# chungimungi/GMLM

Measured on AMD Instinct MI355X. Metric: nodes/sec fwd+bwd (full-batch GraphTextLM step), higher is better.
Workload: dtype bf16; 1 GPU; squirrel-size synthetic graph x1 (N=5201, E=217073, F_in=2089), hidden_channels=768, BERT geometry 768x12, 1257 active text nodes, 16..128 tokens, plm_batch_size=4096; global_nodes=5201, parallelism=single GPU, activation_checkpointing=False, plm_gradient_checkpointing=False, world=1, hip_graph=False, gemm_algorithms=library picks from gmlm_amd/tunable/gfx950.csv (TunableOp lookup)

## Files before the change

gmlm_amd/_lib.py:

```python
from __future__ import annotations

import ctypes as C
import os

_HERE = os.path.dirname(os.path.abspath(__file__))
LIB_PATH = os.path.join(_HERE, "libgmlm_hip.so")

F32, BF16 = 0, 1
_p, _i64, _i32, _f32, _u64, _sz = C.c_void_p, C.c_int64, C.c_int, C.c_float, C.c_uint64, C.c_size_t

SIGNATURES = {
    "gmlm_version": (C.c_int, []),
    "gmlm_last_error": (C.c_char_p, []),
    "gmlm_device_check": (C.c_int, [_p, _p, C.c_char_p, _i32]),
    "gmlm_degree_i32": (C.c_int, [_p, _i64, _i64, _p, _p]),
    "gmlm_degree_f32": (C.c_int, [_p, _i64, _i64, _p, _p]),
    "gmlm_edge_bucket": (C.c_int, [_p, _p, _i64, _i64, _p, _p]),
    "gmlm_relation_histogram": (C.c_int, [_p, _i64, _i32, _p, _p]),
    "gmlm_segment_sort_workspace_bytes": (_sz, [_i64]),
    "gmlm_segment_sort": (C.c_int, [_p, _p, _p, _i32, _i64, _i64, _p, _p, _p, _p, _p, _sz, _p]),
    "gmlm_gather_i64_to_i32": (C.c_int, [_p, _p, _i64, _p, _p]),
    "gmlm_gather_i32": (C.c_int, [_p, _p, _i64, _p, _p]),
    "gmlm_segment_inv_count": (C.c_int, [_p, _i64, _p, _p]),
    "gmlm_split_plan_capacity": (C.c_int, [_i64, _i64, C.POINTER(C.c_int64), C.POINTER(C.c_int64)]),
    "gmlm_split_plan_build": (C.c_int, [_p, _i64, _i64, _i64, _p, _p, _p, _p]),
    "gmlm_rgcn_mean_spmm": (C.c_int, [_p, _i64, _i64, _p, _p, _p, _i32, _i64, _i64, _p, _i64, _i32, _i64, _p, _p, _p, _i64, _i64,
                                      _p, _p]),
    "gmlm_basis_compose_fwd": (C.c_int, [_p, _p, _i32, _i32, _i64, _p, _p]),
    "gmlm_basis_compose_bwd_workspace_bytes": (_sz, [_i32, _i32, _i64]),
    "gmlm_basis_compose_bwd": (C.c_int, [_p, _p, _p, _i32, _i32, _i64, _p, _p, _p, _sz, _p]),
    "gmlm_colstats_workspace_bytes": (_sz, [_i64, _i64]),
    "gmlm_colstats": (C.c_int, [_p, _i32, _p, _i64, _i64, _p, _p, _p, _sz, _p]),
    "gmlm_graphnorm_finalize": (C.c_int, [_p, _p, _p, _p, _i64, _i64, _f32, _p, _p, _p]),
    "gmlm_graphnorm_apply": (C.c_int, [_p, _p, _p, _p, _p, _p, _i64, _i64, _i32, _f32, _u64, _p, _p, _i32, _p]),
    "gmlm_graphnorm_bwd_stats": (C.c_int, [_p, _i32, _p, _p, _p, _p, _p, _p, _i64, _i64, _i32, _f32, _u64, _p, _p, _p, _sz, _p]),
    "gmlm_graphnorm_bwd_apply": (C.c_int, [_p, _i32, _p, _p, _p, _p, _p, _p, _p, _i64, _i64, _i64, _i32, _f32, _u64, _p,
                                           _p, _p, _p, _p, _p]),
    "gmlm_bias_res_layernorm_fwd": (C.c_int, [_p, _p, _p, _p, _p, _i64, _i64, _f32, _i32, _f32, _u64, _p, _p, _p, _p, _i32, _p]),
    "gmlm_layernorm_bwd_workspace_bytes": (_sz, [_i64, _i64]),
    "gmlm_bias_res_layernorm_bwd": (C.c_int, [_p, _p, _p, _p, _p, _p, _p, _p, _i64, _i64, _i32, _f32, _u64, _p, _p, _p, _p, _p,
                                              _p, _i32, _p, _sz, _p]),
    "gmlm_attention_fwd": (C.c_int, [_p, _p, _p, _p, _i64, _i64, _i64, _i64, _i64, _i64, _i64, _i64, _f32, _f32, _u64, _p,
                                     _p, _p, _p, _i32, _p, _i64, _p, _i64, _p]),
    "gmlm_attention_bwd_workspace_bytes": (_sz, [_i64, _i64, _i64, _i64, _i64]),
    "gmlm_attention_bwd": (C.c_int, [_p, _p, _p, _p, _p, _p, _p, _i64, _i64, _i64, _i64, _i64, _i64, _i64, _i64, _f32,
                                     _f32, _u64, _p, _p, _p, _p, _i64, _i64, _i64, _i32, _p, _i64, _p, _sz, _p, _p, _p, _p, _i64, _p]),
    "gmlm_embed_sum_fwd": (C.c_int, [_p, _p, _p, _p, _p, _i64, _i64, _i64, _i64, _p, _i32, _p, _p]),
    "gmlm_meanpool_scatter_fwd": (C.c_int, [_p, _p, _p, _i64, _i64, _i64, _p, _i32, _p, _p]),
    "gmlm_meanpool_scatter_bwd": (C.c_int, [_p, _p, _p, _i64, _i64, _i64, _p, _i32, _p, _p]),
    "gmlm_softmask_blend_fwd": (C.c_int, [_p, _p, _p, _f32, _i64, _i64, _p, _i64, _i32, _p]),
    "gmlm_softmask_blend_bwd": (C.c_int, [_p, _i64, _p, _f32, _i64, _i64, _p, _p, _sz, _p]),
    "gmlm_bias_gelu_fwd": (C.c_int, [_p, _p, _i64, _i64, _f32, _u64, _p, _p, _i32, _p]),
    "gmlm_bias_gelu_bwd_workspace_bytes": (_sz, [_i64, _i64, _i32]),
    "gmlm_bias_gelu_bwd": (C.c_int, [_p, _p, _p, _i64, _i64, _f32, _u64, _p, _p, _p, _i32, _p, _sz, _p]),
}


class GmlmHipError(RuntimeError):
    pass


_lib = None


def lib() -> C.CDLL:
    global _lib
    if _lib is not None:
        return _lib
    if not os.path.exists(LIB_PATH):
        raise GmlmHipError(
            f"{LIB_PATH} not found: the HIP extension is not built. Run `make -C gmlm_amd/csrc` "
            "(or __graft_entry__.build()). gmlm_amd has no CPU / eager fallback.")
    handle = C.CDLL(LIB_PATH)
    for name, (res, args) in SIGNATURES.items():
        fn = getattr(handle, name)
        fn.restype, fn.argtypes = res, args
    if handle.gmlm_version() != 1:
        raise GmlmHipError(f"ABI version mismatch: library {handle.gmlm_version()} != binding 1")
    _lib = handle
    return handle


def check(rc: int, what: str = "") -> None:
    if rc != 0:
        msg = lib().gmlm_last_error().decode(errors="replace")
        raise GmlmHipError(f"{what or 'gmlm call'} failed (code {rc}): {msg}")


_device_ok = {}


def require_gfx950(device_index: int) -> None:
    if _device_ok.get(device_index):
        return
    import torch
    with torch.cuda.device(device_index):
        arch = C.create_string_buffer(64)
        cu, wave = C.c_int(0), C.c_int(0)
        check(lib().gmlm_device_check(C.byref(cu), C.byref(wave), arch, 64), "gmlm_device_check")
    _device_ok[device_index] = (cu.value, wave.value, arch.value.decode())


def device_info(device_index: int = 0):
    require_gfx950(device_index)
    return _device_ok[device_index]
```

gmlm_amd/nn.py:

```python
from __future__ import annotations

import math
from typing import Optional

import torch
import torch.nn as nn
import torch.nn.functional as F

from . import ops
from .graph import GraphCache, RelCSR

_GRAPHS = GraphCache(capacity=8)


def compute_dtype(module_dtype: Optional[torch.dtype] = None) -> torch.dtype:
    if module_dtype is not None:
        return module_dtype
    if torch.is_autocast_enabled("cuda"):
        if torch.get_autocast_dtype("cuda") == torch.float16:
            _warn_fp16_once()
        return torch.bfloat16
    return torch.float32


_FP16_WARNED = False


def _warn_fp16_once() -> None:
    global _FP16_WARNED
    if not _FP16_WARNED:
        _FP16_WARNED = True
        import warnings
        warnings.warn("gmlm_amd: fp16 autocast is executed with bf16 operands (the HIP kernels' reduced precision); "
                      "use torch.amp.autocast('cuda', dtype=torch.bfloat16) to make that explicit", stacklevel=3)


def _glorot(t: torch.Tensor) -> None:
    a = math.sqrt(6.0 / (t.size(-2) + t.size(-1)))
    with torch.no_grad():
        t.uniform_(-a, a)


def _linear(x, weight, bias=None):
    sh = _SHADOW
    if sh is not None and x.dtype == sh.dtype:
        wc = sh.get(id(weight))
        bc = sh.get(id(bias)) if bias is not None else None
        if wc is not None and (bias is None or bc is not None):
            return _mm(x, wc, bc, (weight,) + ((bias,) if bias is not None else ()))
    with torch.autocast("cuda", enabled=False):
        w = weight.to(x.dtype)
        b = None if bias is None else bias.to(x.dtype)
        return F.linear(x, w, b)


_F32_OUT = [True]
_F32_MM = [True]


_SLICES_MEASURED = {(2304, 768): 14, (3072, 768): 14, (768, 3072): 14}
SPLITK_ROW_QUANTUM = 112


def _splitk_wgrad(dy2: torch.Tensor, x2: torch.Tensor, keep_fp32: bool = False) -> torch.Tensor:
    t, n = dy2.shape
    k = x2.shape[1]
    tiles = ((n + 255) // 256) * ((k + 255) // 256)
    s = 1
    if tiles < 128 and t >= 16384:
        import math
        s = _SLICES_MEASURED.get((n, k), 16) if t >= 65536 else min(16, max(1, 2 ** round(math.log2(200.0 / tiles))))
    if s == 1:
        if keep_fp32 and dy2.dtype != torch.float32 and _F32_MM[0]:
            try:
                return torch.mm(dy2.t(), x2, out_dtype=torch.float32)
            except (RuntimeError, TypeError):
                _F32_MM[0] = False
        dw = dy2.t() @ x2
        return dw.float() if keep_fp32 else dw
    q = t // s
    a = dy2[:s * q].view(s, q, n).transpose(1, 2)
    b = x2[:s * q].view(s, q, k)
    if _F32_OUT[0] and dy2.dtype != torch.float32:
        try:
            dw = torch.bmm(a, b, out_dtype=torch.float32).sum(0)
        except (RuntimeError, TypeError):
            _F32_OUT[0] = False
            dw = torch.bmm(a, b).float().sum(0)
    else:
        dw = torch.bmm(a, b).float().sum(0)
    if s * q < t:
        dw += dy2[s * q:].t() @ x2[s * q:]
    return dw if keep_fp32 else dw.to(dy2.dtype)


class _Linear(torch.autograd.Function):

    @staticmethod
    def forward(ctx, x, wc, bc, residual, bias_grad, *masters):
        ctx.save_for_backward(x, wc)
        ctx.masters = masters
        ctx.has_bias = bc is not None and bias_grad
        ctx.n_w = len(masters) // 2 if ctx.has_bias else len(masters)
        y = torch.nn.functional.linear(x, wc, bc)
        return (y, x.view_as(x)) if residual else y

    @staticmethod
    def backward(ctx, dy, dxres=None):
        x, wc = ctx.saved_tensors
        masters, n_w = ctx.masters, ctx.n_w
        dy2 = dy.reshape(-1, dy.shape[-1])
        x2 = x.reshape(-1, x.shape[-1])
        dx = None
        if ctx.needs_input_grad[0]:
            if dxres is None:
                dx = (dy2 @ wc).view(x.shape)
            else:
                dres2 = dxres.reshape(-1, x.shape[-1])
                dx = (dres2.addmm_(dy2, wc) if dres2.is_contiguous() else torch.addmm(dres2, dy2, wc)).view(x.shape)
        grads = [None] * len(masters)
        need = ctx.needs_input_grad[5:]
        if any(need[:n_w]):
            dw = _splitk_wgrad(dy2, x2, keep_fp32=True)
            for i, (m, g) in enumerate(zip(masters[:n_w], dw.split([m.shape[0] for m in masters[:n_w]], 0))):
                if need[i]:
                    grads[i] = g if g.dtype == m.dtype else g.to(m.dtype)
        if ctx.has_bias and any(need[n_w:]):
            db = ops.column_sum(dy2) if dy2.is_cuda and dy2.dtype in (torch.float32, torch.bfloat16) else dy2.sum(0, dtype=torch.float32)
            for i, (m, g) in enumerate(zip(masters[n_w:], db.split([m.shape[0] for m in masters[n_w:]], 0))):
                if need[n_w + i]:
                    grads[n_w + i] = g if g.dtype == m.dtype else g.to(m.dtype)
        return (dx, None, None, None, None, *grads)


def _mm(x, wc, bc, masters, residual=False, bias_grad=True):
    with torch.autocast("cuda", enabled=False):
        return _Linear.apply(x, wc, bc, residual, bias_grad, *masters)


class ParamShadow:

    def __init__(self, specs, dtype, device):
        total, plan = 0, []
        for key, masters, pad in specs:
            rows = sum(m.shape[0] for m in masters) + pad
            tail = tuple(masters[0].shape[1:])
            numel = rows
            for d in tail:
                numel *= d
            plan.append((key, masters, (rows,) + tail, total, numel))
            total += (numel + 127) // 128 * 128
        self.dtype = dtype
        with torch.no_grad():
            flat = torch.zeros(total, dtype=dtype, device=device)
            self.flat = flat
            self.views, dsts, srcs = {}, [], []
            for key, masters, shape, off, numel in plan:
                v = flat[off:off + numel].view(shape)
                self.views[key] = v
                r0 = 0
                for m in masters:
                    dsts.append(v[r0:r0 + m.shape[0]])
                    srcs.append(m.detach())
                    r0 += m.shape[0]
            if dsts:
                torch._foreach_copy_(dsts, srcs)

    def get(self, key):
        return self.views.get(key)

    def record_stream(self, stream) -> None:
        if self.flat.is_cuda:
            self.flat.record_stream(stream)


_SHADOW: Optional[ParamShadow] = None


class shadow_params:

    def __init__(self, specs, dtype, device):
        self.args = (specs, dtype, device)
        self.prev = None

    def __enter__(self):
        global _SHADOW
        self.prev = _SHADOW
        specs, dtype, device = self.args
        _SHADOW = ParamShadow(specs, dtype, device) if (dtype != torch.float32 and device.type == "cuda") else None
        return _SHADOW

    def __exit__(self, *exc):
        global _SHADOW
        _SHADOW = self.prev
        return False


class use_shadow:

    def __init__(self, sh):
        self.sh, self.prev = sh, None

    def __enter__(self):
        global _SHADOW
        self.prev = _SHADOW
        if _SHADOW is None:
            _SHADOW = self.sh
        return _SHADOW

    def __exit__(self, *exc):
        global _SHADOW
        _SHADOW = self.prev
        return False


def linear_specs(*mods):
    out = []
    for m in mods:
        out.append((id(m.weight), [m.weight], 0))
        if m.bias is not None:
            out.append((id(m.bias), [m.bias], 0))
    return out


class _RootAddmm(torch.autograd.Function):

    @staticmethod
    def forward(ctx, x, rootc, bc, root, bias):
        ctx.save_for_backward(x, rootc)
        ctx.rows = root.shape[0]
        return torch.addmm(bc, x, rootc)

    @staticmethod
    def backward(ctx, dy):
        x, rootc = ctx.saved_tensors
        dx = dy @ rootc.t() if ctx.needs_input_grad[0] else None
        droot = _splitk_wgrad(x, dy, keep_fp32=True)[:ctx.rows] if ctx.needs_input_grad[3] else None
        db = ops.column_sum(dy) if ctx.needs_input_grad[4] else None
        return dx, None, None, droot, db


class _SelectRows(torch.autograd.Function):

    @staticmethod
    def forward(ctx, x, idx):
        ctx.save_for_backward(idx)
        ctx.rows = x.shape[0]
        return x.index_select(0, idx)

    @staticmethod
    def backward(ctx, g):
        (idx,) = ctx.saved_tensors
        out = g.new_zeros((ctx.rows,) + tuple(g.shape[1:]))
        out.index_copy_(0, idx, g)
        return out, None


class _BasisCompose(torch.autograd.Function):

    @staticmethod
    def forward(ctx, comp_a, weight2d, reducer):
        comp_a, weight2d = comp_a.detach().float().contiguous(), weight2d.detach().float().contiguous()
        ra, nb = comp_a.shape
        cols = weight2d.shape[1]
        ctx.save_for_backward(comp_a, weight2d)
        ctx.reducer = reducer
        if not weight2d.is_cuda or nb > 32 or ra > 5 or cols % 4:
            if not weight2d.is_cuda:
                raise ops._lib.GmlmHipError("gmlm_amd ops run on the GPU only; there is no CPU path")
            ctx.hip = False
            return comp_a @ weight2d
        ctx.hip = True
        w = torch.empty(ra, cols, dtype=torch.float32, device=weight2d.device)
        ops.check(ops.lib().gmlm_basis_compose_fwd(ops._ptr(comp_a), ops._ptr(weight2d), ra, nb, cols, ops._ptr(w),
                                                   ops._stream()), "gmlm_basis_compose_fwd")
        return w

    @staticmethod
    def backward(ctx, dw):
        comp_a, weight2d = ctx.saved_tensors
        dw = dw.float().contiguous()
        if ctx.reducer is not None:
            ctx.reducer(dw)
        if not ctx.hip:
            return dw @ weight2d.t(), comp_a.t() @ dw, None
        ra, nb = comp_a.shape
        cols = weight2d.shape[1]
        dweight = torch.empty_like(weight2d)
        dcomp = torch.empty_like(comp_a)
        ws = ops._ws(ops.lib().gmlm_basis_compose_bwd_workspace_bytes(ra, nb, cols), dw.device)
        ops.check(ops.lib().gmlm_basis_compose_bwd(ops._ptr(comp_a), ops._ptr(weight2d), ops._ptr(dw), ra, nb, cols,
                                                   ops._ptr(dweight), ops._ptr(dcomp), ops._ptr(ws), ws.numel(), ops._stream()),
                  "gmlm_basis_compose_bwd")
        return dcomp, dweight, None


class RGCNConv(nn.Module):

    def __init__(self, in_channels: int, out_channels: int, num_relations: int, num_bases: Optional[int] = None, **kw):
        super().__init__()
        if kw:
            raise TypeError(f"unsupported RGCNConv options: {sorted(kw)}")
        if num_bases is None:
            raise NotImplementedError("only the basis-decomposed form used by the reference (num_bases=30) is implemented")
        self.in_channels, self.out_channels = in_channels, out_channels
        self.num_relations, self.num_bases = num_relations, num_bases
        self.weight = nn.Parameter(torch.empty(num_bases, in_channels, out_channels))
        self.comp = nn.Parameter(torch.empty(num_relations, num_bases))
        self.root = nn.Parameter(torch.empty(in_channels, out_channels))
        self.bias = nn.Parameter(torch.zeros(out_channels))
        self.reset_parameters()

    def reset_parameters(self):
        _glorot(self.weight), _glorot(self.comp), _glorot(self.root)
        nn.init.zeros_(self.bias)

    def relation_weights(self, csr: RelCSR, dtype, in_pad: int = 0, reducer=None) -> torch.Tensor:
        comp = _SelectRows.apply(self.comp, csr.active_index)
        w = _BasisCompose.apply(comp, self.weight.view(self.num_bases, -1), reducer)
        self.weight._gmlm_grad_reduced = self.comp._gmlm_grad_reduced = reducer is not None
        w = w.view(len(csr.active_relations), self.in_channels, self.out_channels)
        if in_pad:
            w = F.pad(w, (0, 0, 0, in_pad))
        return w.reshape(-1, self.out_channels).to(dtype)

    def forward_csr(self, x: torch.Tensor, csr: RelCSR, reducer=None, halo_wait=None) -> torch.Tensor:
        in_pad = x.shape[1] - self.in_channels
        n = csr.num_nodes
        sh = _SHADOW
        rootc = sh.get(id(self.root)) if (sh is not None and x.dtype == sh.dtype) else None
        bc = sh.get(id(self.bias)) if rootc is not None else None
        with torch.autocast("cuda", enabled=False):
            w = self.relation_weights(csr, x.dtype, in_pad, reducer)
            if bc is not None and rootc.shape[0] == x.shape[1]:
                out = _RootAddmm.apply(x if x.shape[0] == n else x[:n], rootc, bc, self.root, self.bias)
            else:
                root = self.root if not in_pad else F.pad(self.root, (0, 0, 0, in_pad))
                out = torch.addmm(self.bias.to(x.dtype), x[:n], root.to(x.dtype))
        if halo_wait is not None:
            x = halo_wait(x)
        h = ops.RGCNAggregate.apply(x, csr)
        with torch.autocast("cuda", enabled=False):
            return out.addmm_(h, w)

    def forward(self, x, edge_index, edge_type):
        csr = _GRAPHS.get(edge_index, x.size(0), self.num_relations, edge_type)
        cd = compute_dtype()
        return self.forward_csr(x.to(cd).contiguous(), csr)


class GraphNorm(nn.Module):

    def __init__(self, in_channels: int, eps: float = 1e-5):
        super().__init__()
        self.in_channels, self.eps = in_channels, eps
        self.weight = nn.Parameter(torch.ones(in_channels))
        self.bias = nn.Parameter(torch.zeros(in_channels))
        self.mean_scale = nn.Parameter(torch.ones(in_channels))

    def forward(self, x, batch=None, *, act: bool = False, dropout_p: float = 0.0, out_dtype=None, reducer=None,
                n_total=None):
        if batch is not None:
            raise NotImplementedError("GraphNorm over several graphs (batch vector) is outside the hot path")
        p = float(dropout_p) if self.training else 0.0
        return ops.GraphNormAct.apply(x, self.weight, self.bias, self.mean_scale, self.eps, act, p,
                                      ops.draw_seed() if p > 0 else 0, out_dtype or torch.float32, reducer, n_total)

# ... 193 lines not shown
```

gmlm_amd/ops.py:

```python
from __future__ import annotations

from typing import Optional

import torch

from . import _lib
from ._lib import BF16, F32, check, lib


def _ptr(t: Optional[torch.Tensor]):
    return None if t is None else t.data_ptr()


def _stream():
    return torch.cuda.current_stream().cuda_stream


def _dt(t: torch.Tensor) -> int:
    if t.dtype == torch.float32:
        return F32
    if t.dtype == torch.bfloat16:
        return BF16
    raise TypeError(f"gmlm_amd kernels take float32 or bfloat16 tensors, got {t.dtype}")


def _cuda(*ts):
    for t in ts:
        if t is not None and not t.is_cuda:
            raise _lib.GmlmHipError("gmlm_amd ops run on the GPU only (tensor on %s); there is no CPU path" % t.device)
    dev = next(t for t in ts if t is not None).device
    _lib.require_gfx950(dev.index if dev.index is not None else torch.cuda.current_device())


def _ws(nbytes: int, device) -> torch.Tensor:
    return torch.empty(max(int(nbytes), 16), dtype=torch.uint8, device=device)


def _f32c(t: torch.Tensor) -> torch.Tensor:
    return t.detach().float().contiguous()


class KernelTimer:

    def __init__(self):
        self.records = []

    def span(self, name, **meta):
        return _Span(self, name, meta)

    def summary(self):
        torch.cuda.synchronize()
        out = {}
        for name, e0, e1, meta in self.records:
            d = out.setdefault(name, dict(launches=0, ms=0.0, bytes=0.0, flops=0.0))
            d["launches"] += 1
            d["ms"] += e0.elapsed_time(e1)
            d["bytes"] += meta.get("bytes", 0.0)
            d["flops"] += meta.get("flops", 0.0)
        return out


class _Span:
    def __init__(self, timer, name, meta):
        self.timer, self.name, self.meta = timer, name, meta

    def __enter__(self):
        self.e0 = torch.cuda.Event(enable_timing=True)
        self.e1 = torch.cuda.Event(enable_timing=True)
        self.e0.record()
        return self

    def __exit__(self, *exc):
        self.e1.record()
        self.timer.records.append((self.name, self.e0, self.e1, self.meta))
        return False


class _NoSpan:
    def __enter__(self):
        return self

    def __exit__(self, *exc):
        return False


TIMER: Optional[KernelTimer] = None
_NOSPAN = _NoSpan()


def _span(name, **meta):
    return TIMER.span(name, **meta) if TIMER is not None else _NOSPAN


def spmm_algorithmic_bytes(num_edges, num_segments, out_rows, f, elem, edge_w=False):
    return float(num_edges * (f * elem + 4 + (4 if edge_w else 0)) + (num_segments + 1) * 4 + out_rows * f * elem)


SEED_DEVICE: Optional[torch.Tensor] = None


def _sd():
    return None if SEED_DEVICE is None else SEED_DEVICE.data_ptr()


def draw_seed() -> int:
    return int(torch.randint(0, 2 ** 62, (1,), device="cpu").item())


def degree(index: torch.Tensor, num_nodes: Optional[int] = None, dtype=torch.float32) -> torch.Tensor:
    _cuda(index)
    index = index.to(torch.long).contiguous()
    if num_nodes is None:
        num_nodes = int(index.max().item()) + 1 if index.numel() else 0
    if dtype == torch.float32:
        out = torch.empty(num_nodes, dtype=torch.float32, device=index.device)
        check(lib().gmlm_degree_f32(_ptr(index), index.numel(), num_nodes, _ptr(out), _stream()), "gmlm_degree_f32")
        return out
    out = torch.empty(num_nodes, dtype=torch.int32, device=index.device)
    check(lib().gmlm_degree_i32(_ptr(index), index.numel(), num_nodes, _ptr(out), _stream()), "gmlm_degree_i32")
    return out.to(dtype)


def edge_types_from_degree(edge_index: torch.Tensor, num_nodes: int) -> torch.Tensor:
    _cuda(edge_index)
    src = edge_index[0].to(torch.long).contiguous()
    e = src.numel()
    deg = torch.empty(num_nodes, dtype=torch.int32, device=src.device)
    check(lib().gmlm_degree_i32(_ptr(src), e, num_nodes, _ptr(deg), _stream()), "gmlm_degree_i32")
    et = torch.empty(e, dtype=torch.long, device=src.device)
    check(lib().gmlm_edge_bucket(_ptr(src), _ptr(deg), e, num_nodes, _ptr(et), _stream()), "gmlm_edge_bucket")
    return et


def _spmm(src, rowptr, idx, edge_w, mean, num_segments, f, out, split=None):
    if split is not None and split.n_long > 0:
        partial = torch.empty(split.n_chunks, f, dtype=torch.float32, device=src.device)
        extra = (split.thresh, _ptr(split.long_seg), _ptr(split.chunk_ptr), _ptr(split.chunk_owner), split.n_long,
                 split.n_chunks, _ptr(partial))
    else:
        extra = (0, None, None, None, 0, 0, None)
    check(lib().gmlm_rgcn_mean_spmm(_ptr(src), src.shape[0], src.stride(0), _ptr(rowptr), _ptr(idx), _ptr(edge_w),
                                    1 if mean else 0, num_segments, f, _ptr(out), f, _dt(src), *extra, _stream()),
          "gmlm_rgcn_mean_spmm")


def column_sum(x: torch.Tensor) -> torch.Tensor:
    _cuda(x)
    x = x.contiguous()
    n, f = x.shape
    out = torch.empty(2, f, dtype=torch.float32, device=x.device)
    if n == 0:
        return out[0].zero_()
    ws = _ws(lib().gmlm_colstats_workspace_bytes(n, f), x.device)
    check(lib().gmlm_colstats(_ptr(x), _dt(x), None, n, f, _ptr(out[0]), _ptr(out[1]), _ptr(ws), ws.numel(), _stream()), "gmlm_colstats")
    return out[0]


def device_split_plan(rowptr: torch.Tensor, num_items: int, thresh: int = 64):
    import ctypes
    from .graph import SplitPlan
    cl, cc = ctypes.c_int64(), ctypes.c_int64()
    check(lib().gmlm_split_plan_capacity(int(num_items), int(thresh), ctypes.byref(cl), ctypes.byref(cc)), "gmlm_split_plan_capacity")
    dev = rowptr.device
    long_seg = torch.empty(cl.value, dtype=torch.int32, device=dev)
    chunk_ptr = torch.empty(cl.value + 1, dtype=torch.int32, device=dev)
    chunk_owner = torch.empty(cc.value, dtype=torch.int32, device=dev)
    check(lib().gmlm_split_plan_build(_ptr(rowptr), rowptr.numel() - 1, int(num_items), int(thresh), _ptr(long_seg), _ptr(chunk_ptr),
                                      _ptr(chunk_owner), _stream()), "gmlm_split_plan_build")
    return SplitPlan(int(thresh), long_seg, chunk_ptr, chunk_owner, int(cl.value), int(cc.value))


class RGCNAggregate(torch.autograd.Function):

    @staticmethod
    def forward(ctx, x: torch.Tensor, csr) -> torch.Tensor:
        _cuda(x)
        x = x.contiguous()
        n_src, f = x.shape
        n = csr.num_nodes
        if n_src != csr.num_src:
            raise ValueError(f"x has {n_src} rows but the graph expects {csr.num_src} source rows")
        out = torch.empty(n, csr.r_active * f, dtype=x.dtype, device=x.device)
        with _span("spmm_fwd", bytes=spmm_algorithmic_bytes(csr.num_edges, n * csr.r_active, n * csr.r_active, f,
                                                           x.element_size()), f=f):
            _spmm(x, csr.rowptr, csr.col, None, True, n * csr.r_active, f, out, csr.split)
        ctx.csr, ctx.n_src = csr, x.shape[0]
        return out

    @staticmethod
    def backward(ctx, gh: torch.Tensor):
        csr = ctx.csr
        gh = gh.contiguous()
        n, rf = gh.shape
        f = rf // csr.r_active
        gx = torch.empty(csr.num_src, f, dtype=gh.dtype, device=gh.device)
        with _span("spmm_bwd", bytes=spmm_algorithmic_bytes(csr.num_edges, csr.num_src, csr.num_src, f, gh.element_size(),
                                                           True), f=f):
            _spmm(gh.view(n * csr.r_active, f), csr.t_rowptr, csr.t_seg, csr.inv_cnt, False, csr.num_src, f, gx, csr.t_split)
        return gx, None


class GraphNormAct(torch.autograd.Function):

    @staticmethod
    def forward(ctx, z, weight, bias, mean_scale, eps, act, p, seed, out_dtype, reducer, n_total):
        _cuda(z)
        z = z.to(out_dtype).contiguous()
        n, f = z.shape
        n_total = int(n_total) if n_total else n
        dev = z.device
        w, b, ms = _f32c(weight), _f32c(bias), _f32c(mean_scale)
        st = _stream()
        dt = _dt(z)
        stats = torch.empty(2, f, dtype=torch.float32, device=dev)
        shift = None
        if reducer is None and n > 0:
            shift = z[0].float().contiguous()
        ws = _ws(lib().gmlm_colstats_workspace_bytes(n, f), dev)
        check(lib().gmlm_colstats(_ptr(z), dt, _ptr(shift), n, f, _ptr(stats[0]), _ptr(stats[1]), _ptr(ws), ws.numel(), st),
              "gmlm_colstats")
        if reducer is not None:
            reducer(stats)
            mu = stats[0] / n_total
            shift = (mu * ms).contiguous()
            check(lib().gmlm_colstats(_ptr(z), dt, _ptr(shift), n, f, _ptr(stats[0]), _ptr(stats[1]), _ptr(ws), ws.numel(),
                                      st), "gmlm_colstats")
            reducer(stats)
            mean = mu.contiguous()
            rstd = torch.rsqrt(stats[1] / n_total + eps).contiguous()
        else:
            mean = torch.empty(f, dtype=torch.float32, device=dev)
            rstd = torch.empty(f, dtype=torch.float32, device=dev)
            check(lib().gmlm_graphnorm_finalize(_ptr(stats[0]), _ptr(stats[1]), _ptr(shift), _ptr(ms), n_total, f, eps,
                                                _ptr(mean), _ptr(rstd), st), "gmlm_graphnorm_finalize")
        y = torch.empty(n, f, dtype=out_dtype, device=dev)
        sd = ctx.sd = _sd()
        check(lib().gmlm_graphnorm_apply(_ptr(z), _ptr(mean), _ptr(rstd), _ptr(w), _ptr(b), _ptr(ms), n, f, int(act),
                                         float(p), seed, sd, _ptr(y), dt, st), "gmlm_graphnorm_apply")
        ctx.save_for_backward(z, mean, rstd, w, b, ms)
        ctx.cfg = (int(act), float(p), seed, reducer, n_total)
        return y

    @staticmethod
    def backward(ctx, gy):
        z, mean, rstd, w, b, ms = ctx.saved_tensors
        act, p, seed, reducer, n_total = ctx.cfg
        gy = gy.contiguous().to(z.dtype)
        n, f = z.shape
        dev = z.device
        st = _stream()
        dt = _dt(z)
        gs = torch.empty(2, f, dtype=torch.float32, device=dev)
        ws = _ws(lib().gmlm_colstats_workspace_bytes(n, f), dev)
        sd = ctx.sd
        check(lib().gmlm_graphnorm_bwd_stats(_ptr(gy), dt, _ptr(z), _ptr(mean), _ptr(rstd), _ptr(w), _ptr(b), _ptr(ms),
                                             n, f, act, p, seed, sd, _ptr(gs), _ptr(ws), ws.numel(), st),
              "gmlm_graphnorm_bwd_stats")
        gs_local = gs
        if reducer is not None:
            gs_local = gs.clone()
            reducer(gs)
        dz = torch.empty(n, f, dtype=z.dtype, device=dev)
        if reducer is None:
            dw = torch.empty(f, dtype=torch.float32, device=dev)
            db = torch.empty_like(dw)
            dms = torch.empty_like(dw)
            check(lib().gmlm_graphnorm_bwd_apply(_ptr(gy), dt, _ptr(z), _ptr(mean), _ptr(rstd), _ptr(w), _ptr(b),
                                                 _ptr(ms), _ptr(gs), n, n_total, f, act, p, seed, sd, _ptr(dz), _ptr(dw),
                                                 _ptr(db), _ptr(dms), st), "gmlm_graphnorm_bwd_apply")
        else:
            check(lib().gmlm_graphnorm_bwd_apply(_ptr(gy), dt, _ptr(z), _ptr(mean), _ptr(rstd), _ptr(w), _ptr(b),
                                                 _ptr(ms), _ptr(gs), n, n_total, f, act, p, seed, sd, _ptr(dz), None, None,
                                                 None, st), "gmlm_graphnorm_bwd_apply")
            dw, db = gs_local[1].clone(), gs_local[0].clone()
            m2 = gs[1] / n_total
            sum_oh_local = (z.float().sum(0) - n * mean * ms) * rstd
            dms = -mean * (w * rstd * (gs_local[0] - m2 * sum_oh_local))
        return dz, dw, db, dms, None, None, None, None, None, None, None


class BiasResLayerNorm(torch.autograd.Function):
    @staticmethod
    def forward(ctx, x, bias, residual, gamma, beta, eps, act, p, seed):
        _cuda(x)
        shape = x.shape
        f = shape[-1]
        x2 = x.contiguous().view(-1, f)
        rows = x2.shape[0]
        res2 = None if residual is None else residual.to(x.dtype).contiguous().view(-1, f)
        bf = None if bias is None else _f32c(bias)
        g, b = _f32c(gamma), _f32c(beta)
        y = torch.empty_like(x2)
        mean = torch.empty(rows, dtype=torch.float32, device=x.device)
        rstd = torch.empty_like(mean)
        sd = ctx.sd = _sd()
        check(lib().gmlm_bias_res_layernorm_fwd(_ptr(x2), _ptr(bf), _ptr(res2), _ptr(g), _ptr(b), rows, f, float(eps),
                                                int(act), float(p), seed, sd, _ptr(y), _ptr(mean), _ptr(rstd), _dt(x2), _stream()),
              "gmlm_bias_res_layernorm_fwd")
        ctx.save_for_backward(x2, res2, bf, g, b, mean, rstd)
        ctx.cfg = (int(act), float(p), seed, shape, bias is not None, residual is not None)
        return y.view(shape)

    @staticmethod
    def backward(ctx, gy):
        x2, res2, bf, g, b, mean, rstd = ctx.saved_tensors
        act, p, seed, shape, has_bias, has_res = ctx.cfg
        rows, f = x2.shape
        gy2 = gy.contiguous().view(rows, f).to(x2.dtype)
        dx = torch.empty_like(x2)
        dres = torch.empty_like(x2) if has_res else None
        dg = torch.empty(f, dtype=torch.float32, device=x2.device)
        dbeta = torch.empty_like(dg)
        dbias = torch.empty_like(dg) if has_bias else None
        ws = _ws(lib().gmlm_layernorm_bwd_workspace_bytes(rows, f), x2.device)
        sd = ctx.sd
        check(lib().gmlm_bias_res_layernorm_bwd(_ptr(gy2), _ptr(x2), _ptr(bf), _ptr(res2), _ptr(g), _ptr(b), _ptr(mean),
                                                _ptr(rstd), rows, f, act, p, seed, sd, _ptr(dx), _ptr(dres), _ptr(dg),
                                                _ptr(dbeta), _ptr(dbias), _dt(x2), _ptr(ws), ws.numel(), _stream()),
              "gmlm_bias_res_layernorm_bwd")
        return (dx.view(shape), dbias, None if dres is None else dres.view(shape), dg, dbeta, None, None, None, None)


def bias_res_layernorm(x, bias, residual, gamma, beta, eps=1e-5, act=False, p=0.0, training=False):
    p = float(p) if training else 0.0
    return BiasResLayerNorm.apply(x, bias, residual, gamma, beta, eps, act, p, draw_seed() if p > 0 else 0)


def _rows_view(t: torch.Tensor, h: int, d: int):
    if t.stride(-1) != 1 or t.shape[-1] != h * d:
        raise ValueError("attention operands must be [b, l, h*d] with a contiguous last dim")
    if t.stride(0) != t.shape[1] * t.stride(1) and t.shape[0] > 1:
        raise ValueError("attention operands must have batch stride = l * row stride")
    return t.stride(1)


def _short_path(dtype, d: int, rows: int, pairs: int) -> bool:
    return dtype == torch.bfloat16 and d == 64 and rows <= 128 and pairs >= 512


class Attention(torch.autograd.Function):

    @staticmethod
    def forward(ctx, q, k, v, kv_len, h, scale, p, seed):
        _cuda(q, k, v)
        b, lq, hd = q.shape
        lk = k.shape[1]
        d = hd // h
        qs, ks, vs = _rows_view(q, h, d), _rows_view(k, h, d), _rows_view(v, h, d)
        out = torch.empty(b, lq, hd, dtype=q.dtype, device=q.device)
        lse = torch.empty(b, h, lq, dtype=torch.float32, device=q.device)
        want_lo = q.dtype == torch.bfloat16 and not _short_path(q.dtype, d, max(lq, lk), b * h) and \
            any(t.requires_grad for t in (q, k, v))
        out_lo = torch.empty_like(out) if want_lo else None
        with _span("attn_fwd_d%d" % d, flops=4.0 * b * h * lq * lk * d):
            sd = ctx.sd = _sd()
            check(lib().gmlm_attention_fwd(_ptr(q), _ptr(k), _ptr(v), _ptr(kv_len), b, h, lq, lk, d, qs, ks, vs, float(scale),
                                           float(p), seed, sd, _ptr(out), _ptr(out_lo), _ptr(lse), _dt(q), None, 0, None, 0, _stream()),
                  "gmlm_attention_fwd")
        ctx.save_for_backward(q, k, v, out, lse, kv_len, out_lo)
        ctx.cfg = (h, float(scale), float(p), seed)
        return out

    @staticmethod
    def backward(ctx, gout):
        q, k, v, out, lse, kv_len, out_lo = ctx.saved_tensors
        h, scale, p, seed = ctx.cfg
        b, lq, hd = q.shape
        lk = k.shape[1]
        d = hd // h
        gout = gout.contiguous().to(q.dtype)
        dq = torch.empty(b, lq, hd, dtype=q.dtype, device=q.device)
        dk = torch.empty(b, lk, hd, dtype=q.dtype, device=q.device)
        dv = torch.empty(b, lk, hd, dtype=q.dtype, device=q.device)
        ws = _ws(lib().gmlm_attention_bwd_workspace_bytes(b, h, lq, lk, d), q.device)
        with _span("attn_bwd_d%d" % d, flops=10.0 * b * h * lq * lk * d):
            sd = ctx.sd
            check(lib().gmlm_attention_bwd(_ptr(q), _ptr(k), _ptr(v), _ptr(out), _ptr(gout), _ptr(lse), _ptr(kv_len), b, h,
                                           lq, lk, d, q.stride(1), k.stride(1), v.stride(1), scale, p, seed, sd, _ptr(dq),
                                           _ptr(dk), _ptr(dv), hd, hd, hd, _dt(q), None, 0, _ptr(ws), ws.numel(), None, None,
                                           _ptr(out_lo), None, 0, _stream()),
                  "gmlm_attention_bwd")
        return dq, dk, dv, None, None, None, None, None


class AttentionQKV(torch.autograd.Function):

    @staticmethod
    def forward(ctx, qkv, kv_len, h, scale, p, seed, cu_seqlens, max_len, pair_count=None, groups=None, *bias_masters):
        _cuda(qkv)
        qkv = qkv.contiguous()
        packed = cu_seqlens is not None
        if packed:
            l, hd3 = qkv.shape
            b = cu_seqlens.numel() - 1
        else:
            b, l, hd3 = qkv.shape
        hd = hd3 // 3
        d = hd // h
        q, k, v = qkv[..., :hd], qkv[..., hd:2 * hd], qkv[..., 2 * hd:]
        out = torch.empty(qkv.shape[:-1] + (hd,), dtype=qkv.dtype, device=qkv.device)
        lse = torch.empty((h, l) if packed else (b, h, l), dtype=torch.float32, device=qkv.device)
        flops = 4.0 * h * d * ((float(pair_count) if pair_count else float(max_len) * l) if packed else float(b) * l * l)
        rows = int(max_len) if packed else l
        short = _short_path(qkv.dtype, d, rows, b * h)
        if groups is not None and not (packed and short):
            groups = None
        n_groups = 0 if groups is None else groups.numel() - 1
        out_lo = torch.empty_like(out) if (qkv.dtype == torch.bfloat16 and not short and qkv.requires_grad) else None
        nb = out.numel() * out.element_size()
        with _span("attn_fwd_d%d" % d, flops=flops, bytes=(4 + (1 if out_lo is not None else 0)) * nb):
            sd = ctx.sd = _sd()
            check(lib().gmlm_attention_fwd(_ptr(q), _ptr(k), _ptr(v), _ptr(kv_len), b, h, l, l, d, hd3, hd3, hd3, float(scale),
                                           float(p), seed, sd, _ptr(out), _ptr(out_lo), _ptr(lse), _dt(qkv), _ptr(cu_seqlens),
                                           int(max_len), _ptr(groups), n_groups, _stream()), "gmlm_attention_fwd")
        if short:
            ctx.save_for_backward(qkv, lse, kv_len, cu_seqlens, groups)
        else:
            ctx.save_for_backward(qkv, lse, kv_len, cu_seqlens, groups, out, out_lo)
        ctx.short = short
        ctx.cfg = (h, float(scale), float(p), seed, int(max_len), b, l, flops)
        ctx.bias_shapes = [(m.shape[0], m.dtype) for m in bias_masters]
        return out

    @staticmethod
    def backward(ctx, gout):
        if ctx.short:
            qkv, lse, kv_len, cu_seqlens, groups = ctx.saved_tensors
            out, out_lo = gout, None
        else:
            qkv, lse, kv_len, cu_seqlens, groups, out, out_lo = ctx.saved_tensors
        h, scale, p, seed, max_len, b, l, flops = ctx.cfg
        want_db = bool(ctx.bias_shapes) and any(ctx.needs_input_grad[10:])
        hd3 = qkv.shape[-1]
        hd = hd3 // 3
        d = hd // h
        gout = gout.contiguous().to(qkv.dtype)
        q, k, v = qkv[..., :hd], qkv[..., hd:2 * hd], qkv[..., 2 * hd:]
        dqkv = torch.empty_like(qkv)
        dq, dk, dv = dqkv[..., :hd], dqkv[..., hd:2 * hd], dqkv[..., 2 * hd:]
        ws = _ws(lib().gmlm_attention_bwd_workspace_bytes(1 if cu_seqlens is not None else b, h, l, l, d), qkv.device)
        rows = max_len if cu_seqlens is not None else l
        fused_db = want_db and ctx.short
        n_groups = 0 if groups is None else groups.numel() - 1
        part = db = None
        if fused_db:
            part = _ws(4 * (n_groups or b) * hd3, qkv.device).view(torch.float32)
            db = torch.empty(hd3, dtype=torch.float32, device=qkv.device)
        with _span("attn_bwd_d%d" % d, flops=2.5 * flops, bytes=(7 + (0 if ctx.short else 2)) * qkv.numel() // 3 * qkv.element_size()):
            sd = ctx.sd
            check(lib().gmlm_attention_bwd(_ptr(q), _ptr(k), _ptr(v), _ptr(out), _ptr(gout), _ptr(lse), _ptr(kv_len), b, h,
                                           l, l, d, hd3, hd3, hd3, scale, p, seed, sd, _ptr(dq), _ptr(dk), _ptr(dv), hd3, hd3,
                                           hd3, _dt(qkv), _ptr(cu_seqlens), max_len, _ptr(ws), ws.numel(), _ptr(part), _ptr(db),
                                           _ptr(out_lo), _ptr(groups), n_groups, _stream()),
                  "gmlm_attention_bwd")
        dbs = ()
        if want_db:
            if db is None:
                db = column_sum(dqkv.reshape(-1, hd3))
# ... 217 lines not shown
```

include/gmlm_hip.h:

```cpp
#ifndef GMLM_HIP_H
#define GMLM_HIP_H

#include <stddef.h>
#include <stdint.h>

#ifdef __cplusplus
extern "C" {
#endif

#define GMLM_ABI_VERSION 1

enum gmlm_dtype { GMLM_F32 = 0, GMLM_BF16 = 1 };
enum gmlm_status {
  GMLM_OK = 0,
  GMLM_EINVAL = -1,
  GMLM_EWORKSPACE = -2,
  GMLM_ELAUNCH = -3,
  GMLM_EDEVICE = -4
};

typedef void* gmlm_stream_t;

int gmlm_version(void);
const char* gmlm_last_error(void);
int gmlm_device_check(int* cu_count, int* wave_size, char* arch, int arch_len);

int gmlm_degree_i32(const int64_t* index, int64_t e, int64_t n, int32_t* deg, gmlm_stream_t stream);
int gmlm_degree_f32(const int64_t* index, int64_t e, int64_t n, float* deg, gmlm_stream_t stream);
int gmlm_edge_bucket(const int64_t* src, const int32_t* deg, int64_t e, int64_t n, int64_t* edge_type,
                     gmlm_stream_t stream);
int gmlm_relation_histogram(const int64_t* edge_type, int64_t e, int num_relations, int32_t* rel_count,
                            gmlm_stream_t stream);

size_t gmlm_segment_sort_workspace_bytes(int64_t e);
int gmlm_segment_sort(const int64_t* node, const int64_t* rel, const int32_t* rel_remap, int r_active, int64_t e,
                      int64_t num_segments, int32_t* keys, int32_t* perm, int32_t* rowptr, int32_t* bad_flag,
                      void* workspace, size_t workspace_bytes, gmlm_stream_t stream);
int gmlm_gather_i64_to_i32(const int64_t* src, const int32_t* perm, int64_t e, int32_t* out, gmlm_stream_t stream);
int gmlm_gather_i32(const int32_t* src, const int32_t* perm, int64_t e, int32_t* out, gmlm_stream_t stream);
int gmlm_segment_inv_count(const int32_t* rowptr, int64_t num_segments, float* inv_cnt, gmlm_stream_t stream);

int gmlm_split_plan_capacity(int64_t num_items, int64_t long_threshold, int64_t* cap_long, int64_t* cap_chunks);
int gmlm_split_plan_build(const int32_t* rowptr, int64_t num_segments, int64_t num_items, int64_t long_threshold,
                          int32_t* long_seg, int32_t* chunk_ptr, int32_t* chunk_owner, gmlm_stream_t stream);

int gmlm_rgcn_mean_spmm(const void* src, int64_t src_rows, int64_t src_stride, const int32_t* rowptr,
                        const int32_t* idx, const float* edge_w, int mean, int64_t num_segments, int64_t f,
                        void* out, int64_t out_stride, int dtype, int64_t long_threshold, const int32_t* long_seg,
                        const int32_t* chunk_ptr, const int32_t* chunk_owner, int64_t n_long, int64_t n_chunks,
                        float* partial, gmlm_stream_t stream);

int gmlm_basis_compose_fwd(const float* comp, const float* weight, int r_active, int num_bases, int64_t cols,
                           float* w, gmlm_stream_t stream);
size_t gmlm_basis_compose_bwd_workspace_bytes(int r_active, int num_bases, int64_t cols);
int gmlm_basis_compose_bwd(const float* comp, const float* weight, const float* dw, int r_active, int num_bases,
                           int64_t cols, float* dweight, float* dcomp, void* workspace, size_t workspace_bytes,
                           gmlm_stream_t stream);

size_t gmlm_colstats_workspace_bytes(int64_t n, int64_t f);
int gmlm_colstats(const void* x, int dtype, const float* shift, int64_t n, int64_t f, float* s1, float* s2,
                  void* workspace, size_t workspace_bytes, gmlm_stream_t stream);
int gmlm_graphnorm_finalize(const float* s1, const float* s2, const float* shift, const float* mean_scale,
                            int64_t n_total, int64_t f, float eps, float* mean, float* rstd, gmlm_stream_t stream);
int gmlm_graphnorm_apply(const void* x, const float* mean, const float* rstd, const float* weight,
                         const float* bias, const float* mean_scale, int64_t n, int64_t f, int act,
                         float dropout_p, uint64_t seed, const uint64_t* seed_dev, void* y, int dtype, gmlm_stream_t stream);
int gmlm_graphnorm_bwd_stats(const void* g, int dtype, const void* x, const float* mean, const float* rstd,
                             const float* weight, const float* bias, const float* mean_scale, int64_t n, int64_t f,
                             int act, float dropout_p, uint64_t seed, const uint64_t* seed_dev, float* gs ,
                             void* workspace, size_t workspace_bytes, gmlm_stream_t stream);
int gmlm_graphnorm_bwd_apply(const void* g, int dtype, const void* x, const float* mean, const float* rstd,
                             const float* weight, const float* bias, const float* mean_scale, const float* gs,
                             int64_t n, int64_t n_total, int64_t f, int act, float dropout_p, uint64_t seed, const uint64_t* seed_dev,
                             void* dx, float* dweight, float* dbias, float* dmean_scale, gmlm_stream_t stream);

int gmlm_bias_res_layernorm_fwd(const void* x, const float* bias, const void* residual, const float* gamma,
                                const float* beta, int64_t rows, int64_t f, float eps, int act, float dropout_p,
                                uint64_t seed, const uint64_t* seed_dev, void* y, float* mean, float* rstd, int dtype, gmlm_stream_t stream);
size_t gmlm_layernorm_bwd_workspace_bytes(int64_t rows, int64_t f);
int gmlm_bias_res_layernorm_bwd(const void* dy, const void* x, const float* bias, const void* residual,
                                const float* gamma, const float* beta, const float* mean, const float* rstd,
                                int64_t rows, int64_t f, int act, float dropout_p, uint64_t seed, const uint64_t* seed_dev, void* dx,
                                void* dresidual, float* dgamma, float* dbeta, float* dbias, int dtype,
                                void* workspace, size_t workspace_bytes, gmlm_stream_t stream);

int gmlm_attention_fwd(const void* q, const void* k, const void* v, const int32_t* kv_len, int64_t b, int64_t h,
                       int64_t lq, int64_t lk, int64_t d, int64_t q_stride, int64_t k_stride, int64_t v_stride,
                       float scale, float dropout_p, uint64_t seed, const uint64_t* seed_dev, void* out, void* out_lo, float* lse,
                       int dtype, const int32_t* cu_seqlens, int64_t max_len, const int32_t* seq_groups, int64_t num_groups,
                       gmlm_stream_t stream);
size_t gmlm_attention_bwd_workspace_bytes(int64_t b, int64_t h, int64_t lq, int64_t lk, int64_t d);
int gmlm_attention_bwd(const void* q, const void* k, const void* v, const void* out, const void* dout,
                       const float* lse, const int32_t* kv_len, int64_t b, int64_t h, int64_t lq, int64_t lk,
                       int64_t d, int64_t q_stride, int64_t k_stride, int64_t v_stride, float scale,
                       float dropout_p, uint64_t seed, const uint64_t* seed_dev, void* dq, void* dk, void* dv, int64_t dq_stride,
                       int64_t dk_stride, int64_t dv_stride, int dtype, const int32_t* cu_seqlens, int64_t max_len,
                       void* workspace, size_t workspace_bytes,
                       float* dbias_partial , float* dbias ,
                       const void* out_lo, const int32_t* seq_groups, int64_t num_groups, gmlm_stream_t stream);

int gmlm_embed_sum_fwd(const float* word, const float* pos, const float* type0, const int64_t* tok, const int64_t* pos_ids,
                       int64_t rows, int64_t p, int64_t vocab, int64_t npos, void* out, int dtype, int32_t* bad_flag,
                       gmlm_stream_t stream);

int gmlm_meanpool_scatter_fwd(const void* hs, const int32_t* len, const int64_t* node_idx, int64_t b, int64_t l,
                              int64_t p, float* out, int dtype, const int32_t* cu_seqlens, gmlm_stream_t stream);
int gmlm_meanpool_scatter_bwd(const float* dout, const int32_t* len, const int64_t* node_idx, int64_t b, int64_t l,
                              int64_t p, void* dhs, int dtype, const int32_t* cu_seqlens, gmlm_stream_t stream);

int gmlm_softmask_blend_fwd(const float* x, const uint8_t* mask, const float* token, float beta, int64_t n,
                            int64_t f, void* out, int64_t out_stride, int dtype, gmlm_stream_t stream);
int gmlm_softmask_blend_bwd(const float* dout, int64_t dout_stride, const uint8_t* mask, float beta, int64_t n,
                            int64_t f, float* dtoken, void* workspace, size_t workspace_bytes, gmlm_stream_t stream);

int gmlm_bias_gelu_fwd(const void* x, const float* bias, int64_t rows, int64_t f, float dropout_p, uint64_t seed, const uint64_t* seed_dev,
                       void* y, int dtype, gmlm_stream_t stream);
size_t gmlm_bias_gelu_bwd_workspace_bytes(int64_t rows, int64_t f, int dtype);
int gmlm_bias_gelu_bwd(const void* dy, const void* x, const float* bias, int64_t rows, int64_t f, float dropout_p,
                       uint64_t seed, const uint64_t* seed_dev, void* dx, float* dbias, int dtype, void* workspace, size_t workspace_bytes,
                       gmlm_stream_t stream);

#ifdef __cplusplus
}
#endif
#endif
```

Baseline: 71370 nodes/s.

## Add native split-K bf16 weight-gradient MFMA kernel with async LDS pipeline

Adds a hand-written HIP kernel for the weight-gradient GEMM (dy^T x) on large token counts. It uses 256x256 output tiles, split-K over token slices, a 4-deep global_load_lds pipeline, transposed LDS reads feeding bf16 MFMAs, an XCD-aware block remap, and a combine kernel that reduces the fp32 partials and handles the token tail. It replaces the library/split-K torch path when shapes are eligible, with the aim of cutting wgrad time in the BERT linear layers. The fp32 partial workspace adds memory traffic, and the kernel may be slower than the tuned library GEMM.

```diff
diff --git a/gmlm_amd/_lib.py b/gmlm_amd/_lib.py
--- a/gmlm_amd/_lib.py
+++ b/gmlm_amd/_lib.py
@@ -53,6 +53,8 @@
     "gmlm_bias_gelu_fwd": (C.c_int, [_p, _p, _i64, _i64, _f32, _u64, _p, _p, _i32, _p]),
     "gmlm_bias_gelu_bwd_workspace_bytes": (_sz, [_i64, _i64, _i32]),
     "gmlm_bias_gelu_bwd": (C.c_int, [_p, _p, _p, _i64, _i64, _f32, _u64, _p, _p, _p, _i32, _p, _sz, _p]),
+    "gmlm_wgrad_workspace_bytes": (_sz, [_i64, _i64, _i64, _i32]),
+    "gmlm_wgrad_bf16": (C.c_int, [_p, _i64, _p, _i64, _i64, _i64, _i64, _i32, _p, _i64, _i32, _p, _sz, _p]),
 }
 
 
diff --git a/gmlm_amd/csrc/wgrad_kernels.hip b/gmlm_amd/csrc/wgrad_kernels.hip
--- /dev/null
+++ b/gmlm_amd/csrc/wgrad_kernels.hip
@@ -0,0 +1,209 @@
+#include "attn_common.hpp"
+
+namespace gmlm {
+
+namespace wg {
+constexpr int BT = 32;
+constexpr int TILE = 256;
+constexpr int NW = 8;
+constexpr int NBUF = 4;
+constexpr int IMG = BT * TILE * 2;
+constexpr int STAGE = 2 * IMG;
+constexpr int LDS = NBUF * STAGE;
+constexpr int PIECES = IMG / 1024 / NW;
+constexpr int VM_PER_STAGE = 2 * PIECES;
+__device__ __forceinline__ int swz(int r) { return 2 * ((r & 3) | (((r >> 3) & 1) << 2)); }
+}
+
+struct WgradParams {
+  const bf16_t* dy;
+  const bf16_t* x;
+  float* part;
+  int64_t ld_dy, ld_x, n, k;
+  int32_t stages, splits, tiles_k, tiles, remap;
+};
+
+__device__ __forceinline__ uint32_t wg_src_off(int64_t ld, int w, int lane) {
+  const int row = 2 * w + (lane >> 5), slot = lane & 31;
+  return 2u * (uint32_t)(row * ld + 8 * (slot ^ wg::swz(row)));
+}
+
+__device__ __forceinline__ void wg_dma(const bf16_t* base, uint32_t off, uint32_t lds) {
+  const uint32_t dst = __builtin_amdgcn_readfirstlane(lds);
+  uint32_t keep;
+  asm volatile("s_mov_b32 %0, m0\n\ts_mov_b32 m0, %3\n\ts_nop 0\n\tglobal_load_lds_dwordx4 %1, %2\n\ts_mov_b32 m0, %0"
+               : "=&s"(keep) : "v"(off), "s"(base), "s"(dst) : "memory");
+}
+
+__global__ __launch_bounds__(wg::NW * 64, 1) void wgrad_bf16_kernel(WgradParams p) {
+  using namespace wg;
+  extern __shared__ __attribute__((aligned(1024))) unsigned char smem_dyn[];
+  const uint32_t lds0 = (uint32_t)(size_t)(__attribute__((address_space(3))) void*)smem_dyn;
+  const int tid = threadIdx.x, lane = tid & 63, w = __builtin_amdgcn_readfirstlane(tid >> 6);
+  const uint32_t nwg = gridDim.x, id = blockIdx.x;
+  uint32_t lid = id;
+  if (p.remap) {
+    const uint32_t q = nwg >> 3, r = nwg & 7, xcd = id & 7;
+    lid = (xcd < r ? xcd * (q + 1) : r * (q + 1) + (xcd - r) * q) + (id >> 3);
+  }
+  const int slice = (int)(lid / (uint32_t)p.tiles), tile = (int)(lid % (uint32_t)p.tiles);
+  const int n0 = (tile / p.tiles_k) * TILE, k0 = (tile % p.tiles_k) * TILE;
+  const int st0 = (int)((int64_t)slice * p.stages / p.splits), st1 = (int)((int64_t)(slice + 1) * p.stages / p.splits);
+  const int ns = st1 - st0;
+
+  const uint32_t offa = wg_src_off(p.ld_dy, w, lane), offb = wg_src_off(p.ld_x, w, lane);
+  const bf16_t* ga = p.dy + (int64_t)st0 * BT * p.ld_dy + n0;
+  const bf16_t* gb = p.x + (int64_t)st0 * BT * p.ld_x + k0;
+  const int64_t stepa = (int64_t)BT * p.ld_dy, stepb = (int64_t)BT * p.ld_x;
+  auto issue = [&](int s) {
+    const uint32_t buf = lds0 + (uint32_t)((s % NBUF) * STAGE) + 1024u * (uint32_t)w;
+    const bf16_t* a = ga + s * stepa;
+    const bf16_t* b = gb + s * stepb;
+#pragma unroll
+    for (int k = 0; k < PIECES; ++k) {
+      wg_dma(a + (int64_t)(16 * k) * p.ld_dy, offa, buf + 1024u * (uint32_t)(NW * k));
+      wg_dma(b + (int64_t)(16 * k) * p.ld_x, offb, buf + (uint32_t)IMG + 1024u * (uint32_t)(NW * k));
+    }
+  };
+
+  const int g = lane >> 4, q = (lane >> 2) & 3, pp = lane & 3;
+  const int wr = w >> 2, wc = w & 3;
+  const int row = 8 * g + q, sw = swz(row);
+  const uint32_t rbase = (uint32_t)(row * (TILE * 2)) + 8u * (uint32_t)(pp & 1);
+  uint32_t aoff[8], boff[4];
+#pragma unroll
+  for (int m = 0; m < 8; ++m) aoff[m] = rbase + 16u * (uint32_t)((((wr * 128 + 16 * m) >> 3) + (pp >> 1)) ^ sw);
+#pragma unroll
+  for (int j = 0; j < 4; ++j) boff[j] = (uint32_t)IMG + rbase + 16u * (uint32_t)((((wc * 64 + 16 * j) >> 3) + (pp >> 1)) ^ sw);
+
+  typedef __attribute__((ext_vector_type(4))) float f32x4;
+  f32x4 acc[8][4];
+#pragma unroll
+  for (int m = 0; m < 8; ++m)
+#pragma unroll
+    for (int j = 0; j < 4; ++j) acc[m][j] = f32x4{0.f, 0.f, 0.f, 0.f};
+
+  const int pre = ns < NBUF - 1 ? ns : NBUF - 1;
+  for (int s = 0; s < pre; ++s) issue(s);
+  int issued = pre;
+  for (int s = 0; s < ns; ++s) {
+    const int younger = issued - s - 1;
+    if (younger >= 2) asm volatile("s_waitcnt vmcnt(8)" ::: "memory");
+    else if (younger == 1) asm volatile("s_waitcnt vmcnt(4)" ::: "memory");
+    else asm volatile("s_waitcnt vmcnt(0)" ::: "memory");
+    static_assert(VM_PER_STAGE == 4 && NBUF == 4, "vmcnt immediates above assume 4 per stage and 2 younger stages");
+    __builtin_amdgcn_s_barrier();
+    asm volatile("" ::: "memory");
+    if (issued < ns) { issue(issued); ++issued; }
+    const unsigned char* img = smem_dyn + (s % NBUF) * STAGE;
+    bf16x8 a[8], b[4];
+#pragma unroll
+    for (int j = 0; j < 4; ++j) {
+      const bf16x4 lo = __builtin_amdgcn_ds_read_tr16_b64_v4bf16(GMLM_LDS3(bf16x4, img + boff[j]));
+      const bf16x4 hi = __builtin_amdgcn_ds_read_tr16_b64_v4bf16(GMLM_LDS3(bf16x4, img + boff[j] + 4 * TILE * 2));
+      b[j] = bf16x8{lo[0], lo[1], lo[2], lo[3], hi[0], hi[1], hi[2], hi[3]};
+    }
+#pragma unroll
+    for (int m = 0; m < 8; ++m) {
+      const bf16x4 lo = __builtin_amdgcn_ds_read_tr16_b64_v4bf16(GMLM_LDS3(bf16x4, img + aoff[m]));
+      const bf16x4 hi = __builtin_amdgcn_ds_read_tr16_b64_v4bf16(GMLM_LDS3(bf16x4, img + aoff[m] + 4 * TILE * 2));
+      a[m] = bf16x8{lo[0], lo[1], lo[2], lo[3], hi[0], hi[1], hi[2], hi[3]};
+    }
+#pragma unroll
+    for (int m = 0; m < 8; ++m)
+#pragma unroll
+      for (int j = 0; j < 4; ++j) acc[m][j] = __builtin_amdgcn_mfma_f32_16x16x32_bf16(a[m], b[j], acc[m][j], 0, 0, 0);
+  }
+
+  float* out = p.part + (int64_t)slice * p.n * p.k + (int64_t)(n0 + wr * 128 + 4 * g) * p.k + k0 + wc * 64 + (lane & 15);
+#pragma unroll
+  for (int m = 0; m < 8; ++m)
+#pragma unroll
+    for (int j = 0; j < 4; ++j)
+#pragma unroll
+      for (int r = 0; r < 4; ++r) out[(int64_t)(16 * m + r) * p.k + 16 * j] = acc[m][j][r];
+}
+
+__global__ __launch_bounds__(256) void wgrad_combine_kernel(const float* __restrict__ part, int splits, int64_t n, int64_t k,
+                                                            const bf16_t* __restrict__ dy, int64_t ld_dy, const bf16_t* __restrict__ x,
+                                                            int64_t ld_x, int64_t t_main, int64_t t, float* __restrict__ out,
+                                                            int64_t ld_out) {
+  const int64_t k4 = k >> 2, i = (int64_t)blockIdx.x * 256 + threadIdx.x;
+  if (i >= n * k4) return;
+  const int64_t r = i / k4, c = 4 * (i - r * k4);
+  typedef __attribute__((ext_vector_type(4))) float f32x4;
+  const int64_t nk = n * k;
+  const float* src = part + r * k + c;
+  f32x4 s = *reinterpret_cast<const f32x4*>(src);
+  for (int j = 1; j < splits; ++j) {
+    const f32x4 v = *reinterpret_cast<const f32x4*>(src + j * nk);
+#pragma unroll
+    for (int e = 0; e < 4; ++e) s[e] = __fadd_rn(s[e], v[e]);
+  }
+  for (int64_t tt = t_main; tt < t; ++tt) {
+    const float a = bf16_to_f32(dy[tt * ld_dy + r]);
+    const bf16x4 xb = *reinterpret_cast<const bf16x4*>(x + tt * ld_x + c);
+#pragma unroll
+    for (int e = 0; e < 4; ++e) s[e] = fmaf(a, (float)xb[e], s[e]);
+  }
+  *reinterpret_cast<f32x4*>(out + r * ld_out + c) = s;
+}
+
+}
+
+using namespace gmlm;
+
+namespace {
+int wgrad_splits(int64_t t, int64_t n, int64_t k, int splits) {
+  const int64_t tiles = (n / wg::TILE) * (k / wg::TILE), stages = t / wg::BT;
+  int64_t s = splits > 0 ? splits : 256 / tiles;
+  if (s < 1) s = 1;
+  if (s > stages) s = stages;
+  return (int)s;
+}
+}
+
+extern "C" size_t gmlm_wgrad_workspace_bytes(int64_t t, int64_t n, int64_t k, int splits) {
+  if (t < wg::BT || n <= 0 || k <= 0) return 0;
+  return (size_t)wgrad_splits(t, n, k, splits) * (size_t)n * (size_t)k * sizeof(float);
+}
+
+extern "C" int gmlm_wgrad_bf16(const void* dy, int64_t ld_dy, const void* x, int64_t ld_x, int64_t t, int64_t n, int64_t k,
+                               int splits, float* out, int64_t ld_out, int flags, void* workspace, size_t workspace_bytes,
+                               gmlm_stream_t stream) {
+  GMLM_REQUIRE(dy && x && out && workspace, "wgrad_bf16: null pointer");
+  GMLM_REQUIRE(t >= wg::BT && n > 0 && k > 0, "wgrad_bf16: need t >= %d and n, k > 0 (t=%lld n=%lld k=%lld)", wg::BT, (long long)t,
+               (long long)n, (long long)k);
+  GMLM_REQUIRE(n % wg::TILE == 0 && k % wg::TILE == 0, "wgrad_bf16: n and k must be multiples of %d (n=%lld k=%lld)", wg::TILE,
+               (long long)n, (long long)k);
+  GMLM_REQUIRE(ld_dy >= n && ld_x >= k && ld_out >= k, "wgrad_bf16: row stride smaller than the row");
+  GMLM_REQUIRE(ld_dy % 8 == 0 && ld_x % 8 == 0 && ld_out % 4 == 0, "wgrad_bf16: row strides must keep rows 16-byte aligned");
+  GMLM_REQUIRE(((uintptr_t)dy | (uintptr_t)x | (uintptr_t)out | (uintptr_t)workspace) % 16 == 0,
+               "wgrad_bf16: pointers must be 16-byte aligned");
+  GMLM_REQUIRE(splits >= 0 && (flags & ~GMLM_WGRAD_NO_REMAP) == 0, "wgrad_bf16: bad splits / flags");
+  GMLM_REQUIRE(ld_dy < (1ll << 26) && ld_x < (1ll << 26), "wgrad_bf16: row stride too large");
+  const int s = wgrad_splits(t, n, k, splits);
+  const size_t need = (size_t)s * (size_t)n * (size_t)k * sizeof(float);
+  if (workspace_bytes < need) {
+    set_error("wgrad_bf16: workspace of %zu bytes, need %zu", workspace_bytes, need);
+    return GMLM_EWORKSPACE;
+  }
+  const int64_t tiles_k = k / wg::TILE, tiles = (n / wg::TILE) * tiles_k, stages = t / wg::BT;
+  GMLM_REQUIRE(tiles * s < (1ll << 31) && stages < (1ll << 31), "wgrad_bf16: problem too large");
+  static std::once_flag once;
+  static hipError_t attr = hipSuccess;
+  std::call_once(once, [] {
+    attr = hipFuncSetAttribute(reinterpret_cast<const void*>(&wgrad_bf16_kernel), hipFuncAttributeMaxDynamicSharedMemorySize, wg::LDS);
+  });
+  GMLM_HIP(attr);
+  hipStream_t st = as_stream(stream);
+  WgradParams p{(const bf16_t*)dy, (const bf16_t*)x, (float*)workspace, ld_dy, ld_x, n, k, (int32_t)stages, s, (int32_t)tiles_k,
+                (int32_t)tiles, (flags & GMLM_WGRAD_NO_REMAP) ? 0 : 1};
+  wgrad_bf16_kernel<<<(unsigned)(tiles * s), wg::NW * 64, wg::LDS, st>>>(p);
+  GMLM_LAUNCH_CHECK();
+  const int64_t items = n * (k / 4);
+  wgrad_combine_kernel<<<(unsigned)((items + 255) / 256), 256, 0, st>>>((const float*)workspace, s, n, k, (const bf16_t*)dy, ld_dy,
+                                                                      (const bf16_t*)x, ld_x, stages * wg::BT, t, out, ld_out);
+  GMLM_LAUNCH_CHECK();
+  return GMLM_OK;
+}
diff --git a/gmlm_amd/nn.py b/gmlm_amd/nn.py
--- a/gmlm_amd/nn.py
+++ b/gmlm_amd/nn.py
@@ -60,9 +60,24 @@
 
 _SLICES_MEASURED = {(2304, 768): 14, (3072, 768): 14, (768, 3072): 14}
 SPLITK_ROW_QUANTUM = 112
+NATIVE_WGRAD = True
+NATIVE_WGRAD_MIN_T = 16384
+NATIVE_WGRAD_MIN_TILES = 9
+
+
+def _native_wgrad_ok(dy2: torch.Tensor, x2: torch.Tensor, keep_fp32: bool) -> bool:
+    t, n = dy2.shape
+    k = x2.shape[1]
+    return (NATIVE_WGRAD and keep_fp32 and dy2.is_cuda and dy2.dtype == torch.bfloat16 and x2.dtype == torch.bfloat16
+            and t >= NATIVE_WGRAD_MIN_T and n % ops.WGRAD_TILE == 0 and k % ops.WGRAD_TILE == 0
+            and (n // ops.WGRAD_TILE) * (k // ops.WGRAD_TILE) >= NATIVE_WGRAD_MIN_TILES
+            and dy2.stride(1) == 1 and x2.stride(1) == 1 and dy2.stride(0) % 8 == 0 and x2.stride(0) % 8 == 0
+            and dy2.data_ptr() % 16 == 0 and x2.data_ptr() % 16 == 0)
 
 
 def _splitk_wgrad(dy2: torch.Tensor, x2: torch.Tensor, keep_fp32: bool = False) -> torch.Tensor:
+    if _native_wgrad_ok(dy2, x2, keep_fp32):
+        return ops.wgrad_bf16(dy2, x2)
     t, n = dy2.shape
     k = x2.shape[1]
     tiles = ((n + 255) // 256) * ((k + 255) // 256)
diff --git a/gmlm_amd/ops.py b/gmlm_amd/ops.py
--- a/gmlm_amd/ops.py
+++ b/gmlm_amd/ops.py
@@ -154,6 +154,21 @@
     ws = _ws(lib().gmlm_colstats_workspace_bytes(n, f), x.device)
     check(lib().gmlm_colstats(_ptr(x), _dt(x), None, n, f, _ptr(out[0]), _ptr(out[1]), _ptr(ws), ws.numel(), _stream()), "gmlm_colstats")
     return out[0]
+
+
+WGRAD_TILE = 256
+WGRAD_NO_REMAP = 1
+
+
+def wgrad_bf16(dy: torch.Tensor, x: torch.Tensor, splits: int = 0, flags: int = 0) -> torch.Tensor:
+    _cuda(dy, x)
+    t, n = dy.shape
+    k = x.shape[1]
+    out = torch.empty(n, k, dtype=torch.float32, device=dy.device)
+    ws = _ws(lib().gmlm_wgrad_workspace_bytes(t, n, k, splits), dy.device)
+    check(lib().gmlm_wgrad_bf16(_ptr(dy), dy.stride(0), _ptr(x), x.stride(0), t, n, k, splits, _ptr(out), k, flags, _ptr(ws),
+                                ws.numel(), _stream()), "gmlm_wgrad_bf16")
+    return out
 
 
 def device_split_plan(rowptr: torch.Tensor, num_items: int, thresh: int = 64):
diff --git a/include/gmlm_hip.h b/include/gmlm_hip.h
--- a/include/gmlm_hip.h
+++ b/include/gmlm_hip.h
@@ -120,6 +120,11 @@
                        uint64_t seed, const uint64_t* seed_dev, void* dx, float* dbias, int dtype, void* workspace, size_t workspace_bytes,
                        gmlm_stream_t stream);
 
+#define GMLM_WGRAD_NO_REMAP 1
+size_t gmlm_wgrad_workspace_bytes(int64_t t, int64_t n, int64_t k, int splits);
+int gmlm_wgrad_bf16(const void* dy, int64_t ld_dy, const void* x, int64_t ld_x, int64_t t, int64_t n, int64_t k, int splits,
+                    float* out, int64_t ld_out, int flags, void* workspace, size_t workspace_bytes, gmlm_stream_t stream);
+
 #ifdef __cplusplus
 }
 #endif
```

New measurement: 73250 nodes/s, median of 6. 2.6% higher.
